# davidmilligan/MLVFS

Measured on AMD Instinct MI355X. Metric: Mpix/s, 3584x1320 14-bit unpack+badpix+cs5x5+stripes (fused, stream resident in HBM), higher is better.
Workload: dtype u16/int32

## Files before the change

### mlvfs_amd/csrc/k_frame.hip

```cpp
#include "frame_plan.h"
#include "k_frame_dev.h"

namespace mlv {

template <int METHOD, bool PACKED, int VEC, bool SPREAD>
__global__ __launch_bounds__(256, 4) void k_frame(const FrameArgs a)
{
    constexpr bool CHAIN = METHOD == 5;
    using Smem = SmemT<SPREAD, CHAIN>;
    __shared__ Smem sm;

    const int list_mode = a.list_mode;
    const int wl_n = list_mode ? cold_args()->wl_ctl[0] : 0;
    auto list_done = [&]() {
        KArgs ka = cold_args();
        int *ctl = ka->wl_ctl, *stat = ka->wl_stat;
        if (atomicAdd(&ctl[2], 1) == min((int)gridDim.x, wl_n) - 1) {
            ctl[0] = 0; ctl[1] = 0; ctl[2] = 0;
            if (stat) { __atomic_store_n(stat, ctl[3], __ATOMIC_RELAXED); __threadfence_system(); }
        }
    };
    if (list_mode && (int)blockIdx.x >= wl_n) {
        if (wl_n == 0 && blockIdx.x == 0 && threadIdx.x == 0) {
            KArgs ka = cold_args();
// ... 426 lines not shown
    const uint16_t base = prev;
    for (int j = 0; j < 31; j++) {
        const uint16_t next = entry(32 * b + j + 1);
        const unsigned d = (uint16_t)(next - prev);
        if (d > 1) atomicAdd(bad, 1);
        bits |= (d & 1u) << j;
        prev = next;
    }
    e2d[b] = make_uint2(base, bits);
}
namespace {
constexpr size_t E2R_CACHE = 8;
struct E2rEntry { uint2 *table; unsigned long long used; };
std::mutex g_tables_mu;
std::map<std::pair<int, int>, E2rEntry> g_e2r;
std::map<int, uint2 *> g_e2r_parked;
unsigned long long g_e2r_clock = 0;
}
static int e2r_table(const Device *dev, int black, const uint2 **out, hipStream_t stream)
{
    {
        std::lock_guard<std::mutex> lk(g_tables_mu);
        auto it = g_e2r.find({ dev->id, black });
        if (it != g_e2r.end()) { it->second.used = ++g_e2r_clock; *out = it->second.table; return MLVFS_AMD_OK; }
    }
    uint2 *t = nullptr;
    MLV_HIP(hipMalloc(&t, sizeof(uint2) * (E2D_RECORDS_EXT + 1)));
    int *d_bad = (int *)(t + E2D_RECORDS_EXT);
    int bad = -1;
    (void)hipMemsetAsync(d_bad, 0, sizeof(int), stream);
    hipLaunchKernelGGL(k_build_e2d, dim3((E2D_RECORDS_EXT + 255) / 256), dim3(256), 0, stream, dev->luts.u16, black, t, d_bad);
    (void)hipMemcpyAsync(&bad, d_bad, sizeof(int), hipMemcpyDeviceToHost, stream);
    if (hipGetLastError() != hipSuccess || hipStreamSynchronize(stream) != hipSuccess || bad != 0) {
        (void)hipFree(t);
        set_error("building the output table for black level %d failed", black);
        return MLVFS_AMD_ERR_HIP;
    }
    uint2 *victim = nullptr;
    {
        std::lock_guard<std::mutex> lk(g_tables_mu);
        auto it = g_e2r.find({ dev->id, black });
        if (it != g_e2r.end()) {
            it->second.used = ++g_e2r_clock;
            *out = it->second.table;
            victim = t;
        } else {
            size_t mine = 0;
            auto oldest = g_e2r.end();
            for (auto e = g_e2r.begin(); e != g_e2r.end(); ++e)
                if (e->first.first == dev->id) {
                    mine++;
                    if (oldest == g_e2r.end() || e->second.used < oldest->second.used) oldest = e;
                }
            if (mine >= E2R_CACHE) {
                victim = g_e2r_parked[dev->id];
                g_e2r_parked[dev->id] = oldest->second.table;
                g_e2r.erase(oldest);
            }
            g_e2r[{ dev->id, black }] = E2rEntry{ t, ++g_e2r_clock };
            *out = t;
        }
    }
    if (victim) {
        if (victim != t) (void)hipDeviceSynchronize();
        (void)hipFree(victim);
    }
    return MLVFS_AMD_OK;
}

void launch_frame_p(const FramePlan &pl, int method, bool packed, int vec, bool spread, hipStream_t stream, const FrameArgs &a);
void launch_frame_s(const FramePlan &pl, int method, int vec, bool spread, hipStream_t stream, const FrameArgs &a);

bool frame_kernel_takes(const Geom &g, const void *src, size_t src_stride, const void *dst, size_t dst_stride, int nframes)
{
    if (g.bpp == 14) return true;
    if (g.bpp != 12 && g.bpp != 10) return false;
    const bool aligned = ((uintptr_t)src % 16) == 0 && ((uintptr_t)dst % 16) == 0 && (nframes == 1 || (src_stride % 16 == 0 && dst_stride % 16 == 0));
    return aligned && g.w >= 16 && g.w % (g.bpp == 12 ? 8 : 16) == 0;
}

int launch_frame(const Device *dev, const Geom &g, bool packed, const void *src, size_t src_stride, void *dst,
                 size_t dst_stride, int nframes, int method, const PatchView *pv, bool stripes,
                 const int32_t *coef, hipStream_t stream, bool spread)
// ... 111 lines not shown
```

### mlvfs_amd/csrc/k_frame_dev.h

```cpp
#pragma once
#include "clip.h"
#include <cstdlib>
#include <map>
#include <mutex>
#include <vector>
#include <algorithm>
#include <cstdio>
#include <type_traits>

typedef short mlv_pk16 __attribute__((ext_vector_type(2)));
__device__ __forceinline__ int mlv_min_(int a, int b) { return min(a, b); }
__device__ __forceinline__ int mlv_max_(int a, int b) { return max(a, b); }
__device__ __forceinline__ mlv_pk16 mlv_min_(mlv_pk16 a, mlv_pk16 b) { return __builtin_elementwise_min(a, b); }
__device__ __forceinline__ mlv_pk16 mlv_max_(mlv_pk16 a, mlv_pk16 b) { return __builtin_elementwise_max(a, b); }
#define MLV_NET_FN __device__ __forceinline__
#define mlv_mn(a, b) mlv_min_((a), (b))
#define mlv_mx(a, b) mlv_max_((a), (b))
#include "median_nets.h"


namespace mlv {

constexpr int TCW = FRAME_TCW;
constexpr int TCH = FRAME_TCH;
constexpr int HC = FRAME_HC;
constexpr int PW = TCW + 2 * HC;
constexpr int PH = TCH + 2 * HC;
constexpr int RH = TCH + HC;
constexpr int STRIP = 4;
constexpr int GROUPS = TCW / 4;
constexpr int N_MAIN = TCH * GROUPS;
constexpr int N_ITEMS = N_MAIN + TCH;
constexpr int N_TOP_MAIN = 2 * HC * GROUPS, N_TOP = N_TOP_MAIN + 2 * HC;
constexpr int DARK_ITEMS_MIN = 24;
constexpr int FB_ROBUST = 12;
constexpr int FB_WAIT_MIN = 1, FB_WAIT_MAX = 15;
constexpr int FB_DIRECT = 60;
constexpr int PMAP_WORDS = 64;
static_assert(N_ITEMS <= 255 && TCH * 17 <= 256 && N_TOP <= 128, "one item per thread; 17 median lanes per tile row");

struct FrameArgs {
// ... 21 lines not shown
    int *wl_ctl;
    int list_mode;
    int *wl_stat;
    const int *ev32;
};

typedef int mlv_i32x4 __attribute__((ext_vector_type(4)));
__device__ unsigned short mlv_sbl_u16(mlv_i32x4 rsrc, int vindex, int voffset, int soffset, int aux) __asm("llvm.amdgcn.struct.buffer.load.i16");
typedef unsigned mlv_tab_u32x2 __attribute__((ext_vector_type(2)));
__device__ mlv_tab_u32x2 mlv_sbl_x2(mlv_i32x4 rsrc, int vindex, int voffset, int soffset, int aux) __asm("llvm.amdgcn.struct.buffer.load.v2i32");
__device__ __forceinline__ mlv_i32x4 table_rsrc(const void *p, unsigned stride, unsigned entries)
{
    const unsigned long long a = (unsigned long long)p;
    mlv_i32x4 r;
    r.x = (int)(unsigned)a;
    r.y = (int)(((unsigned)(a >> 32) & 0xFFFFu) | (stride << 16));
    r.z = (int)entries;
    r.w = 0x00020000;
    return r;
}
constexpr int E2R_ENTRIES = 14 * MLV_EV_RES;
constexpr int E2D_RECORDS = E2R_ENTRIES / 32;
constexpr int E2D_RECORDS_EXT = 2 * E2D_RECORDS;
constexpr int AUX_DEFAULT = 0;

constexpr int XCHG_WORDS = 28;
template <bool SPREAD_, bool CHAIN_>
struct __align__(16) SmemT {
    static constexpr bool SPREAD = SPREAD_;
    static constexpr bool CHAIN = CHAIN_;
    uint16_t raw[2 * RH][2 * TCW];
    int dr[PH][PW];
    int db[PH][PW];
    int ge[RH][TCW];
    uint16_t t16[MLV_T16_N + (SPREAD_ ? 64 : 0)];
    uint32_t has_patch[PMAP_WORDS];
    uint32_t xchg[CHAIN_ ? 3 : 1][XCHG_WORDS];
    uint8_t fb_queue[CHAIN_ ? 256 : 4];
    int fb_count;
    int next_tile, next_end;
    int dark_items[2];
    int walk[5];
};
static_assert(sizeof(SmemT<true, true>) <= 40 * 1024, "four workgroups per CU need <= 40 KiB of LDS each");

__device__ __forceinline__ void lds_barrier()
// ... 842 lines not shown
    o.stripes = kt->stripes; o.coef_pk = kt->coef_pk; o.coef_fast = kt->coef_fast; o.white = kt->white;
#pragma unroll
    for (int i = 0; i < 8; i++) o.co[i] = kt->coef[i];
    return o;
}

__device__ __forceinline__ void put_rb(uint32_t &top, uint32_t &bot, uint32_t ur, uint32_t ub, unsigned long long m)
{
    asm("s_mov_b64 vcc, %4\n\t"
        "v_cndmask_b32_sdwa %0, %0, %2, vcc dst_sel:WORD_0 dst_unused:UNUSED_PRESERVE src0_sel:WORD_0 src1_sel:WORD_0\n\t"
        "v_cndmask_b32_sdwa %1, %1, %3, vcc dst_sel:WORD_1 dst_unused:UNUSED_PRESERVE src0_sel:WORD_1 src1_sel:WORD_0"
        : "+v"(top), "+v"(bot) : "v"(ur), "v"(ub), "s"(m) : "vcc");
}
__device__ __forceinline__ unsigned long long lanes_gt(int a, int b) { return __builtin_amdgcn_sicmp(a, b, 38); }
__device__ __forceinline__ unsigned long long lanes_ge(int a, int b) { return __builtin_amdgcn_sicmp(a, b, 39); }
__device__ __forceinline__ unsigned long long lanes_lt(int a, int b) { return __builtin_amdgcn_sicmp(a, b, 40); }

struct NoSmem {};
__device__ __forceinline__ bool smoothed_low(const int (&er)[STRIP], const int (&eb)[STRIP])
{
    const int lo = min(min(min(min(er[0], er[1]), er[2]), min(er[3], eb[0])), min(min(eb[1], eb[2]), eb[3]));
    return __any(lo < 7 * MLV_EV_RES);
}
template <int METHOD, bool PACKED, bool VECST, bool CLAMP, bool XM, bool ANYSTRIPES, bool BRIGHT, class SM, bool RAWREG = false>
__device__ __forceinline__ void strip_output_t(const SM &sm, const OutArgs &oa, int w, int h, int black, int f, int tx0, int ty0, int jj, int kk,
                                               unsigned long long msmooth, const int (&gev)[STRIP], int gev_off, const int (&er)[STRIP], const int (&eb)[STRIP], bool store,
                                               uint32_t *rtop = nullptr, uint32_t *rbot = nullptr)
{
    const int y = ty0 + 2 * jj, x = tx0 + 2 * STRIP * kk;
    uint32_t top[STRIP], bot[STRIP];
    auto read_raw = [&]() {
        if constexpr (RAWREG) {
#pragma unroll
            for (int c = 0; c < STRIP; c++) { top[c] = rtop[c]; bot[c] = rbot[c]; }
        } else {
            const uint4 v0 = *(const uint4 *)&sm.raw[2 * jj][2 * STRIP * kk];
            const uint4 v1 = *(const uint4 *)&sm.raw[2 * jj + 1][2 * STRIP * kk];
            top[0] = v0.x; top[1] = v0.y; top[2] = v0.z; top[3] = v0.w;
            bot[0] = v1.x; bot[1] = v1.y; bot[2] = v1.z; bot[3] = v1.w;
        }
    };
    if (METHOD == 0) read_raw();
    if (METHOD != 0) {
        const mlv_i32x4 rs_e2d = table_rsrc(oa.e2d, 8, E2D_RECORDS_EXT);
        int ur[STRIP], ub[STRIP], cr[STRIP], cb[STRIP];
        mlv_tab_u32x2 dr2[STRIP], db2[STRIP];
#pragma unroll
        for (int c = 0; c < STRIP; c++) {
            cr[c] = CLAMP ? min(max(er[c], 0), MLV_EV_MAX) : er[c];
            cb[c] = CLAMP ? min(max(eb[c], 0), MLV_EV_MAX) : eb[c];
            dr2[c] = mlv_sbl_x2(rs_e2d, cr[c] >> 5, 0, 0, AUX_DEFAULT);
            db2[c] = mlv_sbl_x2(rs_e2d, cb[c] >> 5, 0, 0, AUX_DEFAULT);
        }
        read_raw();
        asm volatile("" :: "v"(dr2[0]), "v"(dr2[1]), "v"(dr2[2]), "v"(dr2[3]), "v"(db2[0]), "v"(db2[1]), "v"(db2[2]), "v"(db2[3]));
#pragma unroll
        for (int c = 0; c < STRIP; c++) {
            ur[c] = (int)(__builtin_popcount(bfe_low_bits(dr2[c].y, (uint32_t)cr[c])) + dr2[c].x);
            ub[c] = (int)(__builtin_popcount(bfe_low_bits(db2[c].y, (uint32_t)cb[c])) + db2[c].x);
        }
#pragma unroll
        for (int c = 0; c < STRIP; c++) {
            unsigned long long okm = msmooth;
            if (!BRIGHT) okm &= lanes_ge((int)((uint32_t)gev[c] - (uint32_t)gev_off), 2 * MLV_EV_RES) & lanes_gt(er[c], MLV_EV_RES) & lanes_gt(eb[c], MLV_EV_RES);
            if (XM) okm &= lanes_ge(x + 2 * c, 4) & lanes_lt(x + 2 * c, w - 4);
            put_rb(top[c], bot[c], (uint32_t)ur[c], (uint32_t)ub[c], okm);
        }
    }
    if (oa.stripes) {
        const int black16 = (int)(uint16_t)black, white16 = (int)(uint16_t)oa.white;
        if (!ANYSTRIPES) stripe_strip_pk<CLAMP>(top, bot, oa.co, black16, white16);
        else if (PACKED && oa.coef_pk) stripe_strip_pk<true>(top, bot, oa.co, black16, white16);
        else if (oa.coef_fast) stripe_strip<true>(top, bot, oa.co, black16, white16);
        else stripe_strip<false>(top, bot, oa.co, black16, white16);
    }
    if constexpr (RAWREG) {
#pragma unroll
        for (int c = 0; c < STRIP; c++) { rtop[c] = top[c]; rbot[c] = bot[c]; }
    }
    if (store && y < h) {
        if (VECST) {
            if (x < w) {
                const uint32_t T = ((uint32_t)ty0 * (uint32_t)w + (uint32_t)tx0) * 2u;
                const mlv_i32x4 rs_out = frame_rsrc(oa.dst + (size_t)f * oa.dst_stride + T, (uint32_t)w * (uint32_t)h * 2u - T);
                const uint32_t vo = (__umul24((uint32_t)(2 * jj), (uint32_t)w) + 2 * STRIP * (uint32_t)kk) * 2u;
                const mlv_u32x4 vt = { top[0], top[1], top[2], top[3] }, vb = { bot[0], bot[1], bot[2], bot[3] };
                mlv_rbs_x4(vt, rs_out, (int)vo, 0, 2);
                if (y + 1 < h) mlv_rbs_x4(vb, rs_out, (int)vo, w * 2, 2);
// ... 62 lines not shown
```

### mlvfs_amd/csrc/k_frame_p.hip

```cpp
#include "frame_plan.h"
#include "k_stream_dev.h"

namespace mlv {

constexpr int P_WAIT_MIN = 1, P_WAIT_MAX = 15;
template <bool SPREAD_>
struct __align__(16) SmemP {
    static constexpr bool SPREAD = SPREAD_;
    uint16_t raw[2 * RH][2 * TCW];
    uint32_t pk[PH][PW];
    int ge[RH][TCW];
    uint16_t t16[MLV_T16_N + (SPREAD_ ? 64 : 0)];
    uint32_t has_patch[PMAP_WORDS];
    uint32_t xchg[3][XCHG_WORDS];
    int unc[2];
    int low[2];
    int dim[2];
    int next_tile, next_end;
    int walk[5];
    int2 carry_at[256];
    uint4 carry_spare;
};

struct PGroup {
// ... 98 lines not shown
    for (int i = 0; i < 4 * NC; i++) tv[i] = *(const uint16_t *)((const char *)t + t16_offset<SPREAD>(fb[i]));
    uint32_t exr[NC], exb[NC], exg[NC];
#pragma unroll
    for (int c = 0; c < NC; c++) { exr[c] = fb[4 * c] >> 8; exb[c] = fb[4 * c + 3] >> 8; exg[c] = (fb[4 * c + 1] + fb[4 * c + 2]) >> 8; }
#pragma unroll
    for (int c = 0; c < NC; c += 2) {
        asm volatile("" :: "v"(exr[c]), "v"(exb[c]), "v"(exg[c]), "v"(exr[c + 1]), "v"(exb[c + 1]), "v"(exg[c + 1]));
    }
#pragma unroll
    for (int i = 0; i < 4 * NC; i += 8) {
        asm volatile("" :: "v"(tv[i]), "v"(tv[i + 1]), "v"(tv[i + 2]), "v"(tv[i + 3]), "v"(tv[i + 4]), "v"(tv[i + 5]), "v"(tv[i + 6]), "v"(tv[i + 7]));
    }
    uint32_t nref_r = 0u - (uint32_t)ref_r, nref_b = 0u - (uint32_t)ref_b;
    asm("" : "+v"(nref_r), "+v"(nref_b));
#pragma unroll
    for (int c = 0; c < NC; c++) {
        const uint32_t gb = add3_u32(exg[c], tv[4 * c + 1], tv[4 * c + 2]) >> 1;
        ge[c] = (int)(gb - (127u << 15));
        uint32_t ngr = nref_r - gb, ngb = nref_b - gb;
        pk[c] = as_u(__builtin_amdgcn_cvt_pk_i16((int)add3_u32(exr[c], tv[4 * c + 0], ngr), (int)add3_u32(exb[c], tv[4 * c + 3], ngb)));
    }
}

template <int NC>
__device__ __forceinline__ void cell_multi_pk_tab(const uint32_t *p0, const uint32_t *p1, uint32_t koff, const int *tab, int ref_r, int ref_b,
                                                  int (&ge)[NC], uint32_t (&pk)[NC])
{
    uint32_t ev[4 * NC];
#pragma unroll
    for (int c = 0; c < NC; c++) {
        const uint32_t px[4] = { p0[2 * c], p0[2 * c + 1], p1[2 * c], p1[2 * c + 1] };
#pragma unroll
        for (int i = 0; i < 4; i++) ev[4 * c + i] = *(const uint32_t *)((const char *)tab + ((px[i] << 2) + koff));
    }
#pragma unroll
    for (int i = 0; i < 4 * NC; i += 8) {
        asm volatile("" :: "v"(ev[i]), "v"(ev[i + 1]), "v"(ev[i + 2]), "v"(ev[i + 3]), "v"(ev[i + 4]), "v"(ev[i + 5]), "v"(ev[i + 6]), "v"(ev[i + 7]));
    }
    uint32_t nref_r = 1u - (uint32_t)ref_r, nref_b = 1u - (uint32_t)ref_b;
#pragma unroll
    for (int c = 0; c < NC; c++) {
        const uint32_t gb = (ev[4 * c + 1] + ev[4 * c + 2]) >> 1;
        ge[c] = (int)gb;
        const uint32_t ng = ~gb;
        pk[c] = as_u(__builtin_amdgcn_cvt_pk_i16((int)add3_u32(ev[4 * c + 0], nref_r, ng), (int)add3_u32(ev[4 * c + 3], nref_b, ng)));
    }
// ... 418 lines not shown
    }
    __syncthreads();
    const int lane = (int)threadIdx.x & 63;
    const int w = a.w, h = a.h, black = a.black;
    const uint32_t koff = 4u - 4u * (uint32_t)black;
    const int rows = h >> 1;
    const StreamGrid sg = stream_grid(cols, segs, fold);
    const int ntasks = cold_args()->nframes * sg.per_frame;
    const uint32_t pitch = (uint32_t)(w >> 3) * 14u;
    int *tickets = cold_args()->tickets;
    uint4 (*const mypark)[2][PARK_LANES] = sm.park[threadIdx.x >> 6];
    const int plane = min(max(lane - 1, 0), PARK_LANES - 1);
    const bool parks = lane >= 1 && lane <= PARK_LANES;
    for (;;) {
        const int task = stream_draw(tickets, lane);
        if (task >= ntasks) break;
        const StreamTask t = stream_task<VEC>(task, sg, segs, seg_rows, fold, S_OUT, lane, w, rows);
        const int f = t.f, c = t.c, j0 = t.j0, j1 = t.j1, nparts = t.nparts, P = t.P, roff = t.roff;
        KArgs kt = cold_args();
        const uint8_t *const frame = kt->src + (size_t)f * kt->src_stride;
        const mlv_i32x4 rs_in = frame_rsrc(frame, kt->src_bytes);
        mlv_i32x4 rs_out = { 0, 0, 0, 0 };
        int tx0 = 0;
        bool xm = false;
        uint32_t dA0[4], dA1[4], dB0[4], dB1[4];
        auto issue = [&](int r, uint32_t (&d0)[4], uint32_t (&d1)[4]) { stream_issue(rs_in, r, roff, rows, pitch, t.gbyte, d0, d1); };
        issue(j0 - 2, dA0, dA1);
        issue(j0 - 1, dB0, dB1);
        int ref_r, ref_b;
        {
            const int x0 = min(max(8 * (c * S_OUT + S_OUT / 2), 0), (w - 16) & ~1), y0 = min(j0 + j1, (h - 4) & ~1) & ~1;
            const uint32_t px = fetch_clamped<BPP>(frame, w, h, x0 + (lane & 15), y0 + (lane >> 4));
            const int ev = sm.ev[1 + min(max((int)px - black, 1), 16383)];
            constexpr int CX[5] = { 0, 3, 6, 1, 5 }, CY[5] = { 0, 0, 0, 1, 1 };
            int sdr[5], sdb[5];
#pragma unroll
            for (int k = 0; k < 5; k++) {
                const int l0 = 2 * CX[k] + 32 * CY[k];
                const int rr = __builtin_amdgcn_readlane(ev, l0), g1 = __builtin_amdgcn_readlane(ev, l0 + 1);
                const int g2 = __builtin_amdgcn_readlane(ev, l0 + 16), bb = __builtin_amdgcn_readlane(ev, l0 + 17);
                const int gg = (g1 + g2) >> 1;
                sdr[k] = rr - gg; sdb[k] = bb - gg;
            }
            auto med5 = [](const int (&v)[5]) { return med3i(v[4], max(min(v[0], v[1]), min(v[2], v[3])), min(max(v[0], v[1]), max(v[2], v[3]))); };
            ref_r = med5(sdr);
            ref_b = med5(sdb);
        }
        int n_pm = 0, pm_cell = -1;
        uint32_t pm_top = 0, pm_bot = 0;
        bool list_all = false;
        if (kt->patch) {
            KArgs ka = kt;
            const int4 *cells = ka->cells + (size_t)f * ka->n_rec;
            const int *toff = ka->tile_off;
            const int tx_n = ka->tiles_x, ty_n = ka->tiles_y;
            const int cx_lo = 4 * (c * S_OUT - 1), cx_hi = cx_lo + 4 * P;
            const int tc0 = max(cx_lo - HC, 0) / TCW, tc1 = min((cx_hi - 1 + HC) / TCW, tx_n - 1);
            for (int q = 0; q < nparts; q++) {
                const int j0q = j0 + q * seg_rows, j1q = min(j0q + seg_rows, rows);
                if (j0q >= rows) break;
                const int cy_lo = j0q - 2, cy_hi = j1q + 2;
                const int tr0 = max(cy_lo, 0) / TCH, tr1 = min((cy_hi - 1) / TCH, ty_n - 1), ntr = tr1 - tr0 + 1;
                constexpr int MAXTR = 6;
                int my_lo = 0, my_hi = 0;
                if (lane < ntr && lane < MAXTR) { my_lo = toff[(tr0 + lane) * tx_n + tc0]; my_hi = toff[(tr0 + lane) * tx_n + tc1 + 1]; }
                if (ntr > MAXTR) list_all = true;
                int4 rec[MAXTR];
#pragma unroll
                for (int i = 0; i < MAXTR; i++) {
// ... 75 lines not shown
            if (smooth_row) {
                PGroup gq;
#pragma unroll
                for (int cc = 0; cc < 4; cc++) {
                    const mlv_pk16 xv[1] = { as_pk(x[cc]) };
                    mlv_insert4(c4[cc], xv, gq.s[cc]);
                }
                mlv_merge55(gq.s[0], gq.s[1], gq.p0);
                mlv_merge55(gq.s[2], gq.s[3], gq.p1);
                mlv_quad_mid6(gq.p0, gq.p1, gq.q);
                PNext n;
                pchain_fetch_lists(gq, n);
                pchain_fetch_window(gq, n);
                mlv_pk16 oc[STRIP];
                pchain_finish(gq, n, oc);
                o[0] = as_pk((uint32_t)dpp_prev_i((int)as_u(oc[2]))); o[1] = as_pk((uint32_t)dpp_prev_i((int)as_u(oc[3])));
                o[2] = oc[0]; o[3] = oc[1];
                const unsigned long long um = __ballot(t.writes && pk_uncertain(o)) & msmooth;
                if (um) { unc_lanes |= um; unc_r0 = min(unc_r0, jr); unc_r1 = max(unc_r1, jr); }
            }
            int er[STRIP], eb[STRIP];
#pragma unroll
            for (int cc = 0; cc < STRIP; cc++) {
                er[cc] = wadd(wadd(gej[cc], ref_r), (int)o[cc].x);
                eb[cc] = wadd(wadd(gej[cc], ref_b), (int)o[cc].y);
            }
            uint32_t top[STRIP], bot[STRIP];
            {
                const uint4 (&slot)[2][PARK_LANES] = mypark[(unsigned)(jr + 2 * SLOTS) % (unsigned)SLOTS];
                const uint4 t4 = slot[0][plane], b4 = slot[1][plane];
                top[0] = t4.x; top[1] = t4.y; top[2] = t4.z; top[3] = t4.w;
                bot[0] = b4.x; bot[1] = b4.y; bot[2] = b4.z; bot[3] = b4.w;
            }
            OutArgs oa = out_args(cold_args());
            oa.e2d = e2d_early; oa.stripes = stripes_early;
            stream_output<5>(oa, t, tx0, xm, rs_out, w, h, black, jr, yl, msmooth, fl, gej, er, eb, top, bot, hook);
        };
        auto named_as_used = [](const uint32_t (&n0)[4], const uint32_t (&n1)[4]) {
            asm volatile("" :: "v"(n0[0]), "v"(n0[1]), "v"(n0[2]), "v"(n0[3]), "v"(n1[0]), "v"(n1[1]), "v"(n1[2]), "v"(n1[3]));
        };
        auto pair_step = [&](auto OUT, int r) {
            int ge0[4], ge1[4];
            uint32_t pk0[4], pk1[4];
            mlv_pk16 c4[4][4];
            auto early_a = [&] { if constexpr (!OUT.value) issue(r + 2, dA0, dA1); };
            auto early_b = [&] { if constexpr (!OUT.value) issue(r + 3, dB0, dB1); };
            auto late_a = [&] { named_as_used(dB0, dB1); issue(r + 2, dA0, dA1); };
            auto late_b = [&] { named_as_used(dA0, dA1); issue(r + 3, dB0, dB1); };
            const int f0 = load_row(r, dA0, dA1, early_a, ge0, pk0);
            if constexpr (OUT.value) {
                sort_common(pkr[1], pkr[2], pkr[3], pk0, c4);
                finish_row(r - 2, c4, pkr[0], f0 | fl1 | fl2 | fl3 | fl4, geA, late_a);
            }
            const int f1 = load_row(r + 1, dB0, dB1, early_b, ge1, pk1);
            if constexpr (OUT.value) finish_row(r - 1, c4, pk1, f1 | f0 | fl1 | fl2 | fl3, geB, late_b);
#pragma unroll
            for (int i = 0; i < 4; i++) { pkr[0][i] = pkr[2][i]; pkr[1][i] = pkr[3][i]; pkr[2][i] = pk0[i]; pkr[3][i] = pk1[i]; geA[i] = ge0[i]; geB[i] = ge1[i]; }
            fl4 = fl2; fl3 = fl1; fl2 = f0; fl1 = f1;
        };
        auto single_step = [&](int r, const uint32_t (&d0)[4], const uint32_t (&d1)[4]) {
            int ge0[4];
            uint32_t pk0[4];
            mlv_pk16 c4[4][4];
            const int f0 = load_row(r, d0, d1, [] {}, ge0, pk0);
            sort_common(pkr[1], pkr[2], pkr[3], pk0, c4);
            finish_row(r - 2, c4, pkr[0], f0 | fl1 | fl2 | fl3 | fl4, geA, StreamNoHook());
#pragma unroll
            for (int i = 0; i < 4; i++) { pkr[0][i] = pkr[1][i]; pkr[1][i] = pkr[2][i]; pkr[2][i] = pkr[3][i]; pkr[3][i] = pk0[i]; geA[i] = geB[i]; geB[i] = ge0[i]; }
            fl4 = fl3; fl3 = fl2; fl2 = fl1; fl1 = f0;
        };
        constexpr std::true_type Y{};
        constexpr std::false_type N{};
        int r = j0 - 2;
#pragma unroll 1
        for (; r < j0 + 2; r += 2) pair_step(N, r);
        named_as_used(dA0, dA1);
        {
            KArgs ko = cold_args();
            rs_out = frame_rsrc(ko->dst + (size_t)f * ko->dst_stride, (uint32_t)w * (uint32_t)h * 2u);
            tx0 = 8 * (c * S_OUT - 1);
            xm = c == 0 || 8 * (c * S_OUT + S_OUT) > w - 4;
        }
#pragma unroll 1
        for (; r < j1; r += 2) pair_step(Y, r);
#pragma unroll 1
        for (bool second = false; r <= j1 + 1; r++, second = true) {
            uint32_t e0[4], e1[4];
#pragma unroll
            for (int i = 0; i < 4; i++) { e0[i] = second ? dB0[i] : dA0[i]; e1[i] = second ? dB1[i] : dA1[i]; }
            single_step(r, e0, e1);
        }
        if (list_all) { unc_lanes = ~0ull; unc_r0 = j0; unc_r1 = j1 - 1; }
        if (unc_lanes && lane == 0) {
            KArgs kl = cold_args();
            const int tnx = kl->tiles_x, tny = kl->tiles_y;
            int *ctl = kl->wl_ctl;
            for (int q = 0; q < nparts; q++) {
                const unsigned long long mq = P == 64 ? unc_lanes : (unc_lanes >> (q * P)) & ((1ull << P) - 1);
                const int r0 = unc_r0 + q * seg_rows, r1 = min(unc_r1 + q * seg_rows, rows - 1);
                if (!mq || r0 >= rows) continue;
                const int l0 = __builtin_ctzll(mq), l1 = 63 - __builtin_clzll(mq);
                const int cx0 = max(4 * (c * S_OUT + l0 - 1), 0), cx1 = min(4 * (c * S_OUT + l1 - 1) + 3, w / 2 - 1);
                const int tc0 = cx0 / TCW, tc1 = min(cx1 / TCW, tnx - 1), tr0 = r0 / TCH, tr1 = min(r1 / TCH, tny - 1);
                for (int tc = tc0; tc <= tc1; tc++) {
// ... 33 lines not shown
```

### mlvfs_amd/csrc/k_frame_s.hip

```cpp
#include "frame_plan.h"
#include "k_stream_dev.h"

namespace mlv {

template <bool SPREAD, int VEC, int METHOD>
__global__ __launch_bounds__(256, 4) void k_frame_s(const FrameArgs a, int cols, int segs, int seg_rows, int fold, int S_OUT)
{
    constexpr int BPP = 14;
    __shared__ __align__(16) uint16_t t16[MLV_T16_N + (SPREAD ? 64 : 0)];
    load_t16_rel<SPREAD>(t16, a.t16, (int)threadIdx.x);
    __syncthreads();
    const int lane = (int)threadIdx.x & 63;
    const int w = a.w, h = a.h, black = a.black;
    const int rows = h >> 1;
    const StreamGrid sg = stream_grid(cols, segs, fold);
    const int ntasks = a.nframes * sg.per_frame;
    const uint32_t pitch = (uint32_t)(w >> 3) * 14u;
    const OutArgs oa = out_args(cold_args());
    int *tickets = a.tickets;
    for (;;) {
        const int task = stream_draw(tickets, lane);
        if (task >= ntasks) break;
        const StreamTask t = stream_task<VEC>(task, sg, segs, seg_rows, fold, S_OUT, lane, w, rows);
        const int f = t.f, j0 = t.j0, j1 = t.j1, roff = t.roff;
        const mlv_i32x4 rs_in = frame_rsrc(a.src + (size_t)f * a.src_stride, a.src_bytes);
        const mlv_i32x4 rs_out = frame_rsrc(oa.dst + (size_t)f * oa.dst_stride, (uint32_t)w * (uint32_t)h * 2u);
        const int tx0 = 8 * (t.c * S_OUT - 1);
        const bool xm = t.c == 0 || 8 * (t.c * S_OUT + S_OUT) > w - 4;

        uint32_t dA0[4], dA1[4], dB0[4], dB1[4];
        auto issue = [&](int r, uint32_t (&d0)[4], uint32_t (&d1)[4]) { stream_issue(rs_in, r, roff, rows, pitch, t.gbyte, d0, d1); };
        int dr2[STRIP] = { 0, 0, 0, 0 }, db2[STRIP] = { 0, 0, 0, 0 };
        int dr1[STRIP] = { 0, 0, 0, 0 }, db1[STRIP] = { 0, 0, 0, 0 }, ge1[STRIP] = { 0, 0, 0, 0 };
        uint32_t top1[STRIP] = { 0, 0, 0, 0 }, bot1[STRIP] = { 0, 0, 0, 0 };
        int flags1 = 3, flags2 = 3;
        int dark_steps = 0;
        issue(j0 - 1, dA0, dA1);
        issue(j0, dB0, dB1);
        auto step = [&](int r, uint32_t (&d0)[4], uint32_t (&d1)[4]) {
            uint32_t p0[8], p1[8];
            unpack8<BPP>(d0, t.sel, t.sel, t.sel, p0);
            unpack8<BPP>(d1, t.sel1, t.sel1, t.sel1, p1);
            if (r + 2 <= j1) issue(r + 2, d0, d1);
            bool dark;
            const int flags0 = stream_row_low(p0, p1, black, dark);
            dark_steps += dark ? 1 : 0;
            int ge[STRIP], dr[STRIP], db[STRIP];
            if (!dark) cell_multi_ev_fast<4, SPREAD>(p0, p1, black, t16, ge, dr, db);
            else {
#pragma unroll
                for (int cc = 0; cc < 4; cc += 2) {
// ... 21 lines not shown
                        mlv_median5(vb, o); eb[cc] = wadd(ge1[cc], o[0]);
                    }
                }
                if (smooth_row && METHOD == 3) {
                    auto med9 = [&](const int (&up)[STRIP], const int (&mid)[STRIP], const int (&dn)[STRIP], int (&e)[STRIP]) {
                        int lo[STRIP + 2], mi[STRIP + 2], hi[STRIP + 2];
#pragma unroll
                        for (int cc = 0; cc < STRIP; cc++) {
                            lo[cc + 1] = min(min(up[cc], mid[cc]), dn[cc]);
                            hi[cc + 1] = max(max(up[cc], mid[cc]), dn[cc]);
                            mi[cc + 1] = med3i(up[cc], mid[cc], dn[cc]);
                        }
                        lo[0] = dpp_prev_i(lo[STRIP]); mi[0] = dpp_prev_i(mi[STRIP]); hi[0] = dpp_prev_i(hi[STRIP]);
                        lo[STRIP + 1] = dpp_next_i(lo[1]); mi[STRIP + 1] = dpp_next_i(mi[1]); hi[STRIP + 1] = dpp_next_i(hi[1]);
#pragma unroll
                        for (int cc = 0; cc < STRIP; cc++)
                            e[cc] = wadd(ge1[cc], med3i(max(max(lo[cc], lo[cc + 1]), lo[cc + 2]), med3i(mi[cc], mi[cc + 1], mi[cc + 2]),
                                                         min(min(hi[cc], hi[cc + 1]), hi[cc + 2])));
                    };
                    med9(dr2, dr1, dr, er);
                    med9(db2, db1, db, eb);
                }
                const unsigned long long msmooth = lanes_ge(yl, 4) & lanes_lt(yl, h - 5);
                stream_output<METHOD>(oa, t, tx0, xm, rs_out, w, h, black, jr, yl, msmooth, flags0 | flags1 | flags2, ge1, er, eb, top1, bot1);
            }
#pragma unroll
            for (int cc = 0; cc < STRIP; cc++) {
                dr2[cc] = dr1[cc]; db2[cc] = db1[cc];
                dr1[cc] = dr[cc]; db1[cc] = db[cc]; ge1[cc] = ge[cc];
                top1[cc] = top[cc]; bot1[cc] = bot[cc];
            }
            flags2 = flags1; flags1 = flags0;
        };
        for (int r = j0 - 1; r <= j1; r += 2) {
            step(r, dA0, dA1);
            if (r + 1 <= j1) step(r + 1, dB0, dB1);
        }
        if (lane == 0 && dark_steps) atomicAdd(&a.wl_ctl[0], dark_steps);
    }
    stream_last_out(tickets, lane, 4, [&] { if (a.wl_stat) { __atomic_store_n(a.wl_stat, a.wl_ctl[0], __ATOMIC_RELAXED); __threadfence_system(); } });
}

void launch_frame_s(const FramePlan &pl, int method, int vec, bool spread, hipStream_t stream, const FrameArgs &a)
{
    with_layout(method, true, vec, spread, [&](auto M, auto P, auto V, auto S) {
        if constexpr ((M.value == 2 || M.value == 3) && P.value && (V.value == 1 || V.value == 2))
            hipLaunchKernelGGL((k_frame_s<S.value, V.value, M.value>), dim3(pl.first_grid), dim3(256), 0, stream, a, pl.cols, pl.segs, pl.seg_rows,
// ... 8 lines not shown
```

### mlvfs_amd/csrc/k_stream_dev.h

```cpp
#pragma once
#include "k_frame_dev.h"

namespace mlv {

struct StreamGrid { int ncols_full, nfolded, per_frame; };
__device__ __forceinline__ StreamGrid stream_grid(int cols, int segs, int fold)
{
    StreamGrid sg;
    sg.ncols_full = fold > 1 ? cols - 1 : cols;
    sg.nfolded = fold > 1 ? (segs + fold - 1) / fold : 0;
    sg.per_frame = sg.ncols_full * segs + sg.nfolded;
    return sg;
}

__device__ __forceinline__ int stream_draw(int *tickets, int lane)
{
    int task = 0;
    if (lane == 0) task = atomicAdd(&tickets[0], 1);
    return __builtin_amdgcn_readfirstlane(task);
}

struct StreamTask {
    int f, c;
    int j0, j1;
// ... 7 lines not shown
template <int VEC>
__device__ __forceinline__ StreamTask stream_task(int task, const StreamGrid &sg, int segs, int seg_rows, int fold, int S_OUT, int lane, int w, int rows)
{
    StreamTask t;
    const int gmax = (w >> 3) - 1;
    t.f = task / sg.per_frame;
    const int rem = task - t.f * sg.per_frame;
    const bool folded = rem >= sg.ncols_full * segs;
    t.c = folded ? sg.ncols_full : rem / segs;
    const int seg = folded ? (rem - sg.ncols_full * segs) * fold : rem - t.c * segs;
    t.j0 = seg * seg_rows; t.j1 = min(t.j0 + seg_rows, rows);
    t.nparts = folded ? fold : 1; t.P = folded ? 64 / fold : 64;
    t.pl = lane & (t.P - 1); t.part = folded ? lane / t.P : 0;
    t.roff = t.part * seg_rows;
    const int g_true = t.c * S_OUT + t.pl - 1;
    t.g = min(max(g_true, 0), gmax);
    t.writes = t.pl >= 1 && t.pl <= min(S_OUT, t.P - 2) && g_true <= gmax && t.j0 + t.roff < rows;
    t.gbyte = (uint32_t)t.g * 14u;
    t.sel = (t.g & 1) ? SEL_MIS : SEL_SWAP;
    t.sel1 = VEC == 2 ? t.sel ^ (SEL_SWAP ^ SEL_MIS) : t.sel;
    return t;
}

__device__ __forceinline__ void stream_issue(mlv_i32x4 rs_in, int r, int roff, int rows, uint32_t pitch, uint32_t gbyte, uint32_t (&d0)[4], uint32_t (&d1)[4])
{
    const int rr = min(max(r + roff, 0), rows - 1);
    const uint32_t o0u = __umul24((uint32_t)(2 * rr), pitch) + gbyte, o0 = o0u & ~3u, o1 = (o0u + pitch) & ~3u;
    const mlv_u32x2 a0 = mlv_rbl_x2(rs_in, (int)o0, 0, AUX_DEFAULT), b0 = mlv_rbl_x2(rs_in, (int)o0 + 8, 0, AUX_DEFAULT);
    const mlv_u32x2 a1 = mlv_rbl_x2(rs_in, (int)o1, 0, AUX_DEFAULT), b1 = mlv_rbl_x2(rs_in, (int)o1 + 8, 0, AUX_DEFAULT);
    d0[0] = a0.x; d0[1] = a0.y; d0[2] = b0.x; d0[3] = b0.y;
    d1[0] = a1.x; d1[1] = a1.y; d1[2] = b1.x; d1[3] = b1.y;
}

__device__ __forceinline__ int stream_row_low(const uint32_t (&p0)[8], const uint32_t (&p1)[8], int black, bool &dark)
{
    uint32_t lo = min(p0[0], p1[0]);
#pragma unroll
    for (int i = 1; i < 8; i++) lo = min(min(lo, p0[i]), p1[i]);
    dark = __any((int)lo <= black);
    int fl = 0;
    if (__any((int)lo <= black + 255)) fl = __any((int)lo <= black + 64) ? 3 : 2;
    return fl;
}

struct StreamNoHook { __device__ __forceinline__ void operator()() const {} };
template <int METHOD, class BEFORE_STORES = StreamNoHook>
__device__ __forceinline__ void stream_output(const OutArgs &oa, const StreamTask &t, int tx0, bool xm, mlv_i32x4 rs_out, int w, int h, int black, int jr, int yl,
                                              unsigned long long msmooth, int fl, const int (&ge)[STRIP], const int (&er)[STRIP], const int (&eb)[STRIP],
                                              uint32_t (&top)[STRIP], uint32_t (&bot)[STRIP], BEFORE_STORES before_stores = BEFORE_STORES())
{
    fl |= oa.stripes && smoothed_low(er, eb) ? 1 : 0;
    auto out = [&](auto CLAMP, auto XM, auto BRIGHT) {
        strip_output_t<METHOD, true, true, CLAMP.value, XM.value, false, BRIGHT.value, NoSmem, true>(NoSmem(), oa, w, h, black, t.f, tx0, 0, jr, t.pl, msmooth,
                                                                                                     ge, 0, er, eb, false, top, bot);
    };
    constexpr std::true_type Y{};
    constexpr std::false_type N{};
    if (fl & 1) { if (xm) out(Y, Y, N); else out(Y, N, N); }
    else if (xm) out(N, Y, N);
    else if (fl == 0) out(N, N, Y);
    else out(N, N, N);
    before_stores();
    if (t.writes) {
        const uint32_t vo = (__umul24((uint32_t)yl, (uint32_t)w) + (uint32_t)(8 * t.g)) * 2u;
        const mlv_u32x4 vt = { top[0], top[1], top[2], top[3] }, vb = { bot[0], bot[1], bot[2], bot[3] };
        mlv_rbs_x4(vt, rs_out, (int)vo, 0, 2);
        mlv_rbs_x4(vb, rs_out, (int)vo, w * 2, 2);
    }
}

template <class AFTER>
__device__ __forceinline__ void stream_last_out(int *tickets, int lane, int waves_per_wg, AFTER after)
{
    if (lane == 0) {
        const int nwaves = (int)gridDim.x * waves_per_wg;
        if (atomicAdd(&tickets[1], 1) == nwaves - 1) {
            tickets[0] = 0; tickets[1] = 0;
            after();
        }
    }
}

}
```

Baseline: 973,100.

## Fold chroma reference into table scalar offset and use lane-mask margins

The METHOD 5 stream path now rounds the per-wave chroma references to multiples of 32 and makes them wave-uniform. The reference is no longer added into every er/eb value. It is applied as a scalar soffset on the e2d table buffer load, which sits inside a new guard-padded allocation, and a single mad_i32_i16 builds each exponent from the packed offset. Horizontal margin handling switches from a per-wave bool that picked the XM template variants to precomputed left and right lane masks, which removes those variants. The risks are a larger, zero-filled table allocation and a rounded reference, which could change outputs slightly if the rounding is not exact.

Result: no change. 977,300 (median of 6 runs) (+0.4%).

```diff
diff --git a/mlvfs_amd/csrc/k_frame.hip b/mlvfs_amd/csrc/k_frame.hip
--- a/mlvfs_amd/csrc/k_frame.hip
+++ b/mlvfs_amd/csrc/k_frame.hip
@@ -472,14 +472,16 @@
     {
         std::lock_guard<std::mutex> lk(g_tables_mu);
         auto it = g_e2r.find({ dev->id, black });
-        if (it != g_e2r.end()) { it->second.used = ++g_e2r_clock; *out = it->second.table; return MLVFS_AMD_OK; }
-    }
+        if (it != g_e2r.end()) { it->second.used = ++g_e2r_clock; *out = it->second.table + E2D_GUARD_RECORDS; return MLVFS_AMD_OK; }
+    }
+    static_assert(e2d_guard_covers(E2D_GUARD_RECORDS, P5_REF_MAX) && E2D_ALLOC_RECORDS == 2 * E2D_GUARD_RECORDS + E2D_RECORDS_EXT,
+                  "a record of the table moved by any reference stays inside the allocation");
     uint2 *t = nullptr;
-    MLV_HIP(hipMalloc(&t, sizeof(uint2) * (E2D_RECORDS_EXT + 1)));
-    int *d_bad = (int *)(t + E2D_RECORDS_EXT);
+    MLV_HIP(hipMalloc(&t, sizeof(uint2) * (E2D_ALLOC_RECORDS + 1)));
+    int *d_bad = (int *)(t + E2D_ALLOC_RECORDS);
     int bad = -1;
-    (void)hipMemsetAsync(d_bad, 0, sizeof(int), stream);
-    hipLaunchKernelGGL(k_build_e2d, dim3((E2D_RECORDS_EXT + 255) / 256), dim3(256), 0, stream, dev->luts.u16, black, t, d_bad);
+    (void)hipMemsetAsync(t, 0, sizeof(uint2) * (E2D_ALLOC_RECORDS + 1), stream);
+    hipLaunchKernelGGL(k_build_e2d, dim3((E2D_RECORDS_EXT + 255) / 256), dim3(256), 0, stream, dev->luts.u16, black, t + E2D_GUARD_RECORDS, d_bad);
     (void)hipMemcpyAsync(&bad, d_bad, sizeof(int), hipMemcpyDeviceToHost, stream);
     if (hipGetLastError() != hipSuccess || hipStreamSynchronize(stream) != hipSuccess || bad != 0) {
         (void)hipFree(t);
@@ -492,7 +494,7 @@
         auto it = g_e2r.find({ dev->id, black });
         if (it != g_e2r.end()) {
             it->second.used = ++g_e2r_clock;
-            *out = it->second.table;
+            *out = it->second.table + E2D_GUARD_RECORDS;
             victim = t;
         } else {
             size_t mine = 0;
@@ -508,7 +510,7 @@
                 g_e2r.erase(oldest);
             }
             g_e2r[{ dev->id, black }] = E2rEntry{ t, ++g_e2r_clock };
-            *out = t;
+            *out = t + E2D_GUARD_RECORDS;
         }
     }
     if (victim) {
diff --git a/mlvfs_amd/csrc/k_frame_dev.h b/mlvfs_amd/csrc/k_frame_dev.h
--- a/mlvfs_amd/csrc/k_frame_dev.h
+++ b/mlvfs_amd/csrc/k_frame_dev.h
@@ -17,6 +17,7 @@
 #define mlv_mn(a, b) mlv_min_((a), (b))
 #define mlv_mx(a, b) mlv_max_((a), (b))
 #include "median_nets.h"
+#include "k_output_math.h"
 
 
 namespace mlv {
@@ -84,6 +85,7 @@
 constexpr int E2R_ENTRIES = 14 * MLV_EV_RES;
 constexpr int E2D_RECORDS = E2R_ENTRIES / 32;
 constexpr int E2D_RECORDS_EXT = 2 * E2D_RECORDS;
+static_assert(OUT_EV_RES == MLV_EV_RES && OUT_E2D_RECORDS_EXT == E2D_RECORDS_EXT, "k_output_math.h restates the table's geometry");
 constexpr int AUX_DEFAULT = 0;
 
 constexpr int XCHG_WORDS = 28;
@@ -972,11 +974,19 @@
     const int lo = min(min(min(min(er[0], er[1]), er[2]), min(er[3], eb[0])), min(min(eb[1], eb[2]), eb[3]));
     return __any(lo < 7 * MLV_EV_RES);
 }
-template <int METHOD, bool PACKED, bool VECST, bool CLAMP, bool XM, bool ANYSTRIPES, bool BRIGHT, class SM, bool RAWREG = false>
+__device__ __forceinline__ bool smoothed_low(const int (&er)[STRIP], const int (&eb)[STRIP], int ref_r, int ref_b)
+{
+    const int lr = min(min(min(er[0], er[1]), er[2]), er[3]), lb = min(min(min(eb[0], eb[1]), eb[2]), eb[3]);
+    return (lanes_lt(lr, wsub(7 * MLV_EV_RES, ref_r)) | lanes_lt(lb, wsub(7 * MLV_EV_RES, ref_b))) != 0;
+}
+template <int METHOD, bool PACKED, bool VECST, bool CLAMP, bool XM, bool ANYSTRIPES, bool BRIGHT, class SM, bool RAWREG = false, bool REF = false>
 __device__ __forceinline__ void strip_output_t(const SM &sm, const OutArgs &oa, int w, int h, int black, int f, int tx0, int ty0, int jj, int kk,
                                                unsigned long long msmooth, const int (&gev)[STRIP], int gev_off, const int (&er)[STRIP], const int (&eb)[STRIP], bool store,
-                                               uint32_t *rtop = nullptr, uint32_t *rbot = nullptr)
-{
+                                               uint32_t *rtop = nullptr, uint32_t *rbot = nullptr, unsigned long long mleft = 0, unsigned long long mright = 0,
+                                               int ref_r = 0, int ref_b = 0)
+{
+    static_assert(!(RAWREG && XM), "the register form takes its margins as lane masks");
+    static_assert(!REF || (RAWREG && !CLAMP), "references apart: the register form's plain and bright variants");
     const int y = ty0 + 2 * jj, x = tx0 + 2 * STRIP * kk;
     uint32_t top[STRIP], bot[STRIP];
     auto read_raw = [&]() {
@@ -992,15 +1002,16 @@
     };
     if (METHOD == 0) read_raw();
     if (METHOD != 0) {
-        const mlv_i32x4 rs_e2d = table_rsrc(oa.e2d, 8, E2D_RECORDS_EXT);
+        const mlv_i32x4 rs_e2d = table_rsrc(REF ? oa.e2d - E2D_GUARD_RECORDS : oa.e2d, 8, E2D_RECORDS_EXT);
+        const int so_r = REF ? e2d_split_offset(ref_r) : 0, so_b = REF ? e2d_split_offset(ref_b) : 0;
         int ur[STRIP], ub[STRIP], cr[STRIP], cb[STRIP];
         mlv_tab_u32x2 dr2[STRIP], db2[STRIP];
 #pragma unroll
         for (int c = 0; c < STRIP; c++) {
             cr[c] = CLAMP ? min(max(er[c], 0), MLV_EV_MAX) : er[c];
             cb[c] = CLAMP ? min(max(eb[c], 0), MLV_EV_MAX) : eb[c];
-            dr2[c] = mlv_sbl_x2(rs_e2d, cr[c] >> 5, 0, 0, AUX_DEFAULT);
-            db2[c] = mlv_sbl_x2(rs_e2d, cb[c] >> 5, 0, 0, AUX_DEFAULT);
+            dr2[c] = mlv_sbl_x2(rs_e2d, cr[c] >> 5, 0, so_r, AUX_DEFAULT);
+            db2[c] = mlv_sbl_x2(rs_e2d, cb[c] >> 5, 0, so_b, AUX_DEFAULT);
         }
         read_raw();
         asm volatile("" :: "v"(dr2[0]), "v"(dr2[1]), "v"(dr2[2]), "v"(dr2[3]), "v"(db2[0]), "v"(db2[1]), "v"(db2[2]), "v"(db2[3]));
@@ -1012,8 +1023,9 @@
 #pragma unroll
         for (int c = 0; c < STRIP; c++) {
             unsigned long long okm = msmooth;
-            if (!BRIGHT) okm &= lanes_ge((int)((uint32_t)gev[c] - (uint32_t)gev_off), 2 * MLV_EV_RES) & lanes_gt(er[c], MLV_EV_RES) & lanes_gt(eb[c], MLV_EV_RES);
+            if (!BRIGHT) okm &= lanes_ge((int)((uint32_t)gev[c] - (uint32_t)gev_off), 2 * MLV_EV_RES) & lanes_gt(er[c], wsub(MLV_EV_RES, ref_r)) & lanes_gt(eb[c], wsub(MLV_EV_RES, ref_b));
             if (XM) okm &= lanes_ge(x + 2 * c, 4) & lanes_lt(x + 2 * c, w - 4);
+            if constexpr (RAWREG) okm &= ~(c < 2 ? mleft : mright);
             put_rb(top[c], bot[c], (uint32_t)ur[c], (uint32_t)ub[c], okm);
         }
     }
diff --git a/mlvfs_amd/csrc/k_frame_p.hip b/mlvfs_amd/csrc/k_frame_p.hip
--- a/mlvfs_amd/csrc/k_frame_p.hip
+++ b/mlvfs_amd/csrc/k_frame_p.hip
@@ -144,6 +144,14 @@
     }
 }
 
+template <int HALF>
+__device__ __forceinline__ int add_half(uint32_t pk, int a)
+{
+    int r;
+    if (HALF) asm("v_mad_i32_i16 %0, %1, 1, %2 op_sel:[1,0,0,0]" : "=v"(r) : "v"(pk), "v"(a));
+    else asm("v_mad_i32_i16 %0, %1, 1, %2" : "=v"(r) : "v"(pk), "v"(a));
+    return r;
+}
 template <int NC>
 __device__ __forceinline__ void cell_multi_pk_tab(const uint32_t *p0, const uint32_t *p1, uint32_t koff, const int *tab, int ref_r, int ref_b,
                                                   int (&ge)[NC], uint32_t (&pk)[NC])
@@ -608,7 +616,7 @@
         const mlv_i32x4 rs_in = frame_rsrc(frame, kt->src_bytes);
         mlv_i32x4 rs_out = { 0, 0, 0, 0 };
         int tx0 = 0;
-        bool xm = false;
+        unsigned long long mleft = 0, mright = 0;
         uint32_t dA0[4], dA1[4], dB0[4], dB1[4];
         auto issue = [&](int r, uint32_t (&d0)[4], uint32_t (&d1)[4]) { stream_issue(rs_in, r, roff, rows, pitch, t.gbyte, d0, d1); };
         issue(j0 - 2, dA0, dA1);
@@ -629,8 +637,8 @@
                 sdr[k] = rr - gg; sdb[k] = bb - gg;
             }
             auto med5 = [](const int (&v)[5]) { return med3i(v[4], max(min(v[0], v[1]), min(v[2], v[3])), min(max(v[0], v[1]), max(v[2], v[3]))); };
-            ref_r = med5(sdr);
-            ref_b = med5(sdb);
+            ref_r = __builtin_amdgcn_readfirstlane(p5_round_ref(med5(sdr)));
+            ref_b = __builtin_amdgcn_readfirstlane(p5_round_ref(med5(sdb)));
         }
         int n_pm = 0, pm_cell = -1;
         uint32_t pm_top = 0, pm_bot = 0;
@@ -752,8 +760,8 @@
             int er[STRIP], eb[STRIP];
 #pragma unroll
             for (int cc = 0; cc < STRIP; cc++) {
-                er[cc] = wadd(wadd(gej[cc], ref_r), (int)o[cc].x);
-                eb[cc] = wadd(wadd(gej[cc], ref_b), (int)o[cc].y);
+                er[cc] = add_half<0>(as_u(o[cc]), gej[cc]);
+                eb[cc] = add_half<1>(as_u(o[cc]), gej[cc]);
             }
             uint32_t top[STRIP], bot[STRIP];
             {
@@ -764,7 +772,7 @@
             }
             OutArgs oa = out_args(cold_args());
             oa.e2d = e2d_early; oa.stripes = stripes_early;
-            stream_output<5>(oa, t, tx0, xm, rs_out, w, h, black, jr, yl, msmooth, fl, gej, er, eb, top, bot, hook);
+            stream_output<5>(oa, t, tx0, mleft, mright, rs_out, w, h, black, jr, yl, msmooth, fl, gej, er, eb, ref_r, ref_b, top, bot, hook);
         };
         auto named_as_used = [](const uint32_t (&n0)[4], const uint32_t (&n1)[4]) {
             asm volatile("" :: "v"(n0[0]), "v"(n0[1]), "v"(n0[2]), "v"(n0[3]), "v"(n1[0]), "v"(n1[1]), "v"(n1[2]), "v"(n1[3]));
@@ -809,7 +817,7 @@
             KArgs ko = cold_args();
             rs_out = frame_rsrc(ko->dst + (size_t)f * ko->dst_stride, (uint32_t)w * (uint32_t)h * 2u);
             tx0 = 8 * (c * S_OUT - 1);
-            xm = c == 0 || 8 * (c * S_OUT + S_OUT) > w - 4;
+            stream_margins(t, S_OUT, w, mleft, mright);
         }
 #pragma unroll 1
         for (; r < j1; r += 2) pair_step(Y, r);
diff --git a/mlvfs_amd/csrc/k_frame_s.hip b/mlvfs_amd/csrc/k_frame_s.hip
--- a/mlvfs_amd/csrc/k_frame_s.hip
+++ b/mlvfs_amd/csrc/k_frame_s.hip
@@ -26,7 +26,8 @@
         const mlv_i32x4 rs_in = frame_rsrc(a.src + (size_t)f * a.src_stride, a.src_bytes);
         const mlv_i32x4 rs_out = frame_rsrc(oa.dst + (size_t)f * oa.dst_stride, (uint32_t)w * (uint32_t)h * 2u);
         const int tx0 = 8 * (t.c * S_OUT - 1);
-        const bool xm = t.c == 0 || 8 * (t.c * S_OUT + S_OUT) > w - 4;
+        unsigned long long mleft, mright;
+        stream_margins(t, S_OUT, w, mleft, mright);
 
         uint32_t dA0[4], dA1[4], dB0[4], dB1[4];
         auto issue = [&](int r, uint32_t (&d0)[4], uint32_t (&d1)[4]) { stream_issue(rs_in, r, roff, rows, pitch, t.gbyte, d0, d1); };
@@ -94,7 +95,7 @@
                     med9(db2, db1, db, eb);
                 }
                 const unsigned long long msmooth = lanes_ge(yl, 4) & lanes_lt(yl, h - 5);
-                stream_output<METHOD>(oa, t, tx0, xm, rs_out, w, h, black, jr, yl, msmooth, flags0 | flags1 | flags2, ge1, er, eb, top1, bot1);
+                stream_output<METHOD>(oa, t, tx0, mleft, mright, rs_out, w, h, black, jr, yl, msmooth, flags0 | flags1 | flags2, ge1, er, eb, 0, 0, top1, bot1);
             }
 #pragma unroll
             for (int cc = 0; cc < STRIP; cc++) {
diff --git a/mlvfs_amd/csrc/k_output_math.h b/mlvfs_amd/csrc/k_output_math.h
--- /dev/null
+++ b/mlvfs_amd/csrc/k_output_math.h
@@ -0,0 +1,43 @@
+#pragma once
+#include <cstdint>
+
+#if defined(__HIPCC__)
+#define MLV_OUT_FN __host__ __device__ inline
+#else
+#define MLV_OUT_FN inline
+#endif
+
+namespace mlv {
+
+MLV_OUT_FN int stream_lane_group(int c, int S_OUT, int pl) { return c * S_OUT + pl - 1; }
+MLV_OUT_FN bool margin_left_lane(int g_true) { return g_true <= 0; }
+MLV_OUT_FN bool margin_right_lane(int g_true, int gmax) { return g_true >= gmax; }
+
+constexpr int OUT_EV_RES = 32768;
+constexpr int OUT_E2D_RECORDS_EXT = 2 * 14 * OUT_EV_RES / 32;
+constexpr int P5_REF_MAX = 14 * OUT_EV_RES;
+constexpr int E2D_GUARD_RECORDS = P5_REF_MAX / 32;
+constexpr bool e2d_guard_covers(int guard_records, int ref_max) { return ref_max % 32 == 0 && ref_max / 32 <= guard_records; }
+constexpr int E2D_ALLOC_RECORDS = E2D_GUARD_RECORDS + OUT_E2D_RECORDS_EXT + E2D_GUARD_RECORDS;
+MLV_OUT_FN int e2d_split_offset(int ref) { return ((ref >> 5) + E2D_GUARD_RECORDS) * 8; }
+
+MLV_OUT_FN int p5_round_ref(int m)
+{
+    const int c = m < -P5_REF_MAX ? -P5_REF_MAX : (m > P5_REF_MAX ? P5_REF_MAX : m);
+    return c & ~31;
+}
+
+struct E2dAt { bool reads; int record; int bits; };
+MLV_OUT_FN E2dAt e2d_at_abs(int er)
+{
+    const uint32_t idx = (uint32_t)(er >> 5);
+    return E2dAt{ idx < (uint32_t)OUT_E2D_RECORDS_EXT, er >> 5, er & 31 };
+}
+MLV_OUT_FN E2dAt e2d_at_split(int e, int ref)
+{
+    const uint32_t idx = (uint32_t)(e >> 5);
+    const bool reads = idx < (uint32_t)OUT_E2D_RECORDS_EXT;
+    return E2dAt{ reads, reads ? (int)idx + e2d_split_offset(ref) / 8 - E2D_GUARD_RECORDS : 0, e & 31 };
+}
+
+}
diff --git a/mlvfs_amd/csrc/k_stream_dev.h b/mlvfs_amd/csrc/k_stream_dev.h
--- a/mlvfs_amd/csrc/k_stream_dev.h
+++ b/mlvfs_amd/csrc/k_stream_dev.h
@@ -1,5 +1,6 @@
 #pragma once
 #include "k_frame_dev.h"
+#include "k_output_math.h"
 
 namespace mlv {
 
@@ -53,6 +54,13 @@
     return t;
 }
 
+__device__ __forceinline__ void stream_margins(const StreamTask &t, int S_OUT, int w, unsigned long long &mleft, unsigned long long &mright)
+{
+    const int g_true = stream_lane_group(t.c, S_OUT, t.pl);
+    mleft = __ballot(margin_left_lane(g_true));
+    mright = __ballot(margin_right_lane(g_true, (w >> 3) - 1));
+}
+
 __device__ __forceinline__ void stream_issue(mlv_i32x4 rs_in, int r, int roff, int rows, uint32_t pitch, uint32_t gbyte, uint32_t (&d0)[4], uint32_t (&d1)[4])
 {
     const int rr = min(max(r + roff, 0), rows - 1);
@@ -76,21 +84,26 @@
 
 struct StreamNoHook { __device__ __forceinline__ void operator()() const {} };
 template <int METHOD, class BEFORE_STORES = StreamNoHook>
-__device__ __forceinline__ void stream_output(const OutArgs &oa, const StreamTask &t, int tx0, bool xm, mlv_i32x4 rs_out, int w, int h, int black, int jr, int yl,
+__device__ __forceinline__ void stream_output(const OutArgs &oa, const StreamTask &t, int tx0, unsigned long long mleft, unsigned long long mright, mlv_i32x4 rs_out, int w, int h, int black, int jr, int yl,
                                               unsigned long long msmooth, int fl, const int (&ge)[STRIP], const int (&er)[STRIP], const int (&eb)[STRIP],
-                                              uint32_t (&top)[STRIP], uint32_t (&bot)[STRIP], BEFORE_STORES before_stores = BEFORE_STORES())
+                                              int ref_r, int ref_b, uint32_t (&top)[STRIP], uint32_t (&bot)[STRIP], BEFORE_STORES before_stores = BEFORE_STORES())
 {
-    fl |= oa.stripes && smoothed_low(er, eb) ? 1 : 0;
-    auto out = [&](auto CLAMP, auto XM, auto BRIGHT) {
-        strip_output_t<METHOD, true, true, CLAMP.value, XM.value, false, BRIGHT.value, NoSmem, true>(NoSmem(), oa, w, h, black, t.f, tx0, 0, jr, t.pl, msmooth,
-                                                                                                     ge, 0, er, eb, false, top, bot);
-    };
+    fl |= oa.stripes && smoothed_low(er, eb, ref_r, ref_b) ? 1 : 0;
     constexpr std::true_type Y{};
     constexpr std::false_type N{};
-    if (fl & 1) { if (xm) out(Y, Y, N); else out(Y, N, N); }
-    else if (xm) out(N, Y, N);
-    else if (fl == 0) out(N, N, Y);
-    else out(N, N, N);
+    if (fl & 1) {
+        int ar[STRIP], ab[STRIP];
+#pragma unroll
+        for (int c = 0; c < STRIP; c++) { ar[c] = wadd(er[c], ref_r); ab[c] = wadd(eb[c], ref_b); }
+        strip_output_t<METHOD, true, true, true, false, false, false, NoSmem, true>(NoSmem(), oa, w, h, black, t.f, tx0, 0, jr, t.pl, msmooth, ge, 0, ar, ab, false,
+                                                                                   top, bot, mleft, mright);
+    } else {
+        auto out = [&](auto BRIGHT) {
+            strip_output_t<METHOD, true, true, false, false, false, BRIGHT.value, NoSmem, true, METHOD == 5>(NoSmem(), oa, w, h, black, t.f, tx0, 0, jr, t.pl, msmooth, ge, 0, er, eb, false,
+                                                                                                top, bot, mleft, mright, ref_r, ref_b);
+        };
+        if (fl == 0) out(Y); else out(N);
+    }
     before_stores();
     if (t.writes) {
         const uint32_t vo = (__umul24((uint32_t)yl, (uint32_t)w) + (uint32_t)(8 * t.g)) * 2u;
```
